# JamesYang007/adelie

Hardware: AMD Instinct MI355X
Metric: lambda-paths/sec (100-lambda grpnet); HBM GB/s vs peak (higher is better)
Workload: dtype f64

## Files before the change

### adelie_amd/csrc/filter_host.hpp

```cpp
#pragma once
#include <algorithm>
#include <cmath>
#include <cstdint>
#include <vector>

namespace ahip {

constexpr int kFilterRuleStrong = 0, kFilterRulePivot = 1;

inline int64_t pivot_need(int64_t old_size, int64_t n_new_active, int64_t G, double subset_ratio, int64_t subset_min,
                          double slack_ratio) {
    const int64_t subset_size =
        std::min<int64_t>(std::max<int64_t>(int64_t(double(old_size) * (1 + subset_ratio)), subset_min), G);
    return subset_size + int64_t(std::ceil(slack_ratio * double(n_new_active))) + old_size + 2;
}

struct FilterRule {
    int screen_rule = kFilterRulePivot;
    double alpha = 1, lm = 0, lm_next = 0;
    bool thr_valid = false;
    double screen_thr = 0;
    int64_t thr_count = 0;
    int64_t G = 0, screen_size = 0, n_new_active = 0;
    double subset_ratio = 0.1, slack_ratio = 1.25;
// ... 8 lines not shown
    } else if (f.screen_rule == kFilterRulePivot) {
        if (!f.thr_valid) return 0;
        if (f.n_new_active > 0) {
            const int64_t need = pivot_need(f.screen_size, f.n_new_active, f.G, f.subset_ratio, f.subset_min, f.slack_ratio);
            if (!(need * 4 < f.G) || double(need) > 0.97 * double(f.thr_count)) return 0;
        }
        tstar = std::min(tstar, f.screen_thr);
    } else {
        return 0;
    }
    return (tstar > 0 && std::isfinite(tstar)) ? tstar : 0;
}

template <class I, class T>
inline std::vector<int32_t> filter_unpenalized_cols(const std::vector<I>& groups, const std::vector<I>& group_sizes,
                                                    const std::vector<T>& penalty) {
    std::vector<int32_t> c;
    for (size_t g = 0; g < groups.size(); ++g)
        if (!(penalty[g] > 0))
            for (I t = 0; t < group_sizes[g]; ++t) c.push_back(int32_t(groups[g] + t));
    return c;
}

constexpr int32_t kFilterOverflow = 1, kFilterStale = 2;
struct FilterFollowUp {
    bool refill;
    bool retire;
};
inline FilterFollowUp filter_follow_up(int32_t flags) {
    return FilterFollowUp{(flags & (kFilterOverflow | kFilterStale)) != 0, (flags & kFilterStale) != 0};
}
inline int64_t filter_list_cap(int64_t p) { return std::max<int64_t>(1024, p / 4); }

}
```

### adelie_amd/csrc/kernels.hpp

```cpp
#pragma once
#include <hip/hip_runtime.h>
#include <cstdint>
#include "gram_shape.hpp"
#include "relu_shape.hpp"
#include "relu_sparse_shape.hpp"
#include "shadow_kind_host.hpp"

namespace ahip {

template <class T>
struct DenseView {
    const T* X;
    int64_t n, p, ld;
};
struct SnpView {
    const uint8_t* bits;
    int64_t n, p, ldb;
};

template <class T>
struct CscView {
    const int64_t* cptr;
    const int32_t* cidx;
    const T* cval;
// ... 28 lines not shown
    const void* X;
    int64_t n, p, ld;
    const double* err;
    const double* nrm;
    int kind = kShadowF32;
    const double* scale = nullptr;
    double fp_term() const { return (4.0 * double(n) + (kind == kShadowQ15 ? 8.0 : 0.0)) * 1.1102230246251565e-16; }
    double elem_bytes() const { return kind == kShadowQ15 ? 2.0 : 4.0; }
};
void launch_shadow_build(const DenseView<double>& X, float* Xs, int64_t lds, double* err, double* nrm, int32_t* bad, hipStream_t s);
int64_t shadow_q15_ld(int64_t n);
void launch_shadow_build_q15(const DenseView<double>& X, int16_t* Xq, int64_t lds, double* scale, double* err, double* nrm,
                             int32_t* bad, hipStream_t s);
int filter_norm_parts(int64_t n);
struct FilteredSweep {
    const double *w, *r;
    double* v;
    double* grad;
    const double *sub_scale, *sub_vec;
    const int32_t* screen_cols;
    int64_t n_screen_cols;
    const int32_t* pen0_cols;
    int64_t n_pen0_cols;
    const int64_t *groups, *group_sizes;
    int64_t G;
    const int32_t* slot;
    const double* penalty;
    double tstar;
    double* sq_part;
    int32_t* list;
    int64_t cap;
    int32_t* meta_i;
    double* meta_d;
    double* work;
};
int64_t filtered_sweep_work_elems(int64_t n, int64_t p, int64_t n_before, int64_t cap);
void enqueue_filtered_sweep(const DenseView<double>& X, const ShadowView& S, const FilteredSweep& a, hipStream_t s);
int64_t sweep_work_elems_csc(int nb, int64_t ncols);
template <class T>
void launch_sweep_csc(const CscView<T>& X, const T* v, T* out, int64_t c0, int64_t ncols, const int32_t* cols,
                      const T* sub_scale, const T* sub_vec, bool square, T* work, hipStream_t s);
constexpr int kVecSumScratch = 8 + 256;
template <class T> void launch_vec_sum(const T* v, int64_t n, T* out, hipStream_t s);
template <class T>
void launch_std_sweep_epilogue(const T* center, const T* inv_scale, const T* raw, const T* raw_plain, const T* vsum, bool square,
                               T* out, int64_t c0, int64_t ncols, const int32_t* cols, const T* sub_scale, const T* sub_vec,
// ... 557 lines not shown
```

### adelie_amd/csrc/kernels_filter.hip

```cpp
#include "sweep_common.hpp"
#include <algorithm>
#include <cfloat>

namespace ahip {

namespace {

__global__ __launch_bounds__(kThreads) void shadow_build_kernel(const double* __restrict__ X, int64_t ld, int64_t n,
                                                                float* __restrict__ Xs, int64_t lds, double* __restrict__ err,
                                                                double* __restrict__ nrm, int32_t* __restrict__ bad) {
    const int64_t j = blockIdx.x;
    const int tid = threadIdx.x;
    const double* col = X + j * ld;
    float* dst = Xs + j * lds;
    double e2 = 0, n2 = 0;
    bool any_bad = false;
    for (int64_t i = tid; i < lds; i += kThreads) {
        float f = 0.f;
        if (i < n) {
            const double x = col[i];
            const bool ok = fabs(x) <= double(FLT_MAX);
            any_bad = any_bad || !ok;
            f = ok ? float(x) : 0.f;
            const double d = x - double(f);
// ... 149 lines not shown

template <int XVEC>
__device__ __forceinline__ void exact_part(const DenseAcc<double>& X, const double* __restrict__ v, int64_t n,
                                           const int32_t* __restrict__ xa, int64_t na, const int32_t* __restrict__ xb,
                                           int64_t nb, int64_t x_rows_per_split, double* __restrict__ stage, double* red) {
    const int64_t ne = na + nb;
    const int64_t c = int64_t(blockIdx.x) % ne;
    const int64_t xsplit = int64_t(blockIdx.x) / ne;
    const int64_t j = c < na ? xa[c] : xb[c - na];
    const int64_t xr0 = xsplit * x_rows_per_split;
    const double s = list_column_sum<XVEC>(X, v, j, xr0, min(n, xr0 + x_rows_per_split), red);
    if (threadIdx.x == 0) stage[xsplit * ne + c] = s;
}

template <class Kind, int XVEC>
__global__ __launch_bounds__(kThreads) void shadow_sweep_kernel(const typename Kind::elem* __restrict__ Xs, int64_t ld,
                                                                const double* __restrict__ scale, const double* __restrict__ v,
                                                                double* __restrict__ out, int64_t n, int64_t ncols,
                                                                int64_t blocks_c, int64_t rows_per_split, int nsplit,
                                                                const double* __restrict__ sub_scale,
                                                                const double* __restrict__ sub_vec, DenseAcc<double> X,
                                                                const int32_t* __restrict__ xa, int64_t na,
                                                                const int32_t* __restrict__ xb, int64_t nb,
                                                                int64_t x_rows_per_split, int x_nsplit, double* __restrict__ stage) {
    constexpr int CB = Kind::CB, VEC = Kind::VEC;
    const int tid = threadIdx.x;
    const int64_t n_exact = (na + nb) * x_nsplit;
    __shared__ double red[kThreads / 64][CB];
    if (int64_t(blockIdx.x) < n_exact) {
        exact_part<XVEC>(X, v, n, xa, na, xb, nb, x_rows_per_split, stage, &red[0][0]);
        return;
    }
    const int64_t b = int64_t(blockIdx.x) - n_exact;
    const int64_t cb = b % blocks_c;
    const int split = int(b / blocks_c);
    const int64_t r0 = int64_t(split) * rows_per_split;
    const int64_t r1 = min(n, r0 + rows_per_split);
    const typename Kind::elem* cp[CB];
#pragma unroll
    for (int k = 0; k < CB; ++k) {
        int64_t c = cb * CB + k;
        if (c >= ncols) c = ncols - 1;
        cp[k] = Xs + c * ld;
    }
    double acc[CB];
#pragma unroll
    for (int k = 0; k < CB; ++k) acc[k] = 0;
    const int64_t body_end = r0 + ((r1 - r0) / VEC) * VEC;
#pragma unroll Kind::kUnroll
    for (int64_t i = r0 + int64_t(tid) * VEC; i < body_end; i += int64_t(kThreads) * VEC) {
        d2_t vv[VEC / 2];
#pragma unroll
        for (int e = 0; e < VEC / 2; ++e) vv[e] = *reinterpret_cast<const d2_t*>(v + i + 2 * e);
        typename Kind::vec xx[CB];
#pragma unroll
        for (int k = 0; k < CB; ++k) xx[k] = __builtin_nontemporal_load(reinterpret_cast<const typename Kind::vec*>(cp[k] + i));
#pragma unroll
        for (int k = 0; k < CB; ++k) {
#pragma unroll
            for (int e = 0; e < VEC; ++e) acc[k] = fma(Kind::row(xx[k], e), vv[e / 2][e % 2], acc[k]);
        }
    }
    for (int64_t i = body_end + tid; i < r1; i += kThreads) {
        const double vi = v[i];
#pragma unroll
        for (int k = 0; k < CB; ++k) acc[k] = fma(double(cp[k][i]), vi, acc[k]);
    }
    panel_epilogue<Kind::kScaled>(acc, red, cb, ncols, 0, nullptr, scale, out, split, nsplit, sub_scale, sub_vec);
}

template <int VEC>
__global__ __launch_bounds__(kThreads) void sweep_list_kernel(DenseAcc<double> X, const double* __restrict__ v,
                                                              double* __restrict__ out, double* __restrict__ part, int64_t n,
                                                              const int32_t* __restrict__ cols, int64_t max_cols,
                                                              const int32_t* __restrict__ count_dev, int64_t rows_per_split,
                                                              int nsplit, const double* __restrict__ sub_scale,
                                                              const double* __restrict__ sub_vec, const double* __restrict__ err,
                                                              const double* __restrict__ nrm, double fp_term,
                                                              const double* __restrict__ vnorm, int32_t* __restrict__ flags) {
    const int64_t c = blockIdx.x;
    const int64_t count = count_dev ? min(int64_t(count_dev[0]), max_cols) : max_cols;
    if (c >= count) return;
    const int split = blockIdx.y;
    const int64_t r0 = int64_t(split) * rows_per_split;
    const int64_t j = cols[c];
    __shared__ double red[kThreads / 64];
    double s = list_column_sum<VEC>(X, v, j, r0, min(n, r0 + rows_per_split), red);
    if (threadIdx.x == 0) {
        if (nsplit == 1) {
            s = centred(s, j, sub_scale, sub_vec);
            if (err) shadow_guard(s, out[j], j, err, nrm, fp_term, vnorm, flags);
// ... 6 lines not shown
__global__ void sweep_list_reduce_kernel(const double* __restrict__ part, double* __restrict__ out,
                                         const int32_t* __restrict__ cols, int64_t max_cols,
                                         const int32_t* __restrict__ count_dev, int nsplit, const double* __restrict__ sub_scale,
                                         const double* __restrict__ sub_vec, const double* __restrict__ err,
                                         const double* __restrict__ nrm, double fp_term, const double* __restrict__ vnorm,
                                         int32_t* __restrict__ flags) {
    const int64_t c = int64_t(blockIdx.x) * blockDim.x + threadIdx.x;
    const int64_t count = count_dev ? min(int64_t(count_dev[0]), max_cols) : max_cols;
    if (c >= count) return;
    const int64_t j = cols[c];
    double s = 0;
    for (int r = 0; r < nsplit; ++r) s += part[int64_t(r) * max_cols + c];
    s = centred(s, j, sub_scale, sub_vec);
    if (err) shadow_guard(s, out[j], j, err, nrm, fp_term, vnorm, flags);
    out[j] = s;
}

constexpr int kClassifyThreads = 1024, kClassifyRun = 6;
__global__ __launch_bounds__(kClassifyThreads) void filter_classify_kernel(
    double* __restrict__ grad, const int64_t* __restrict__ groups, const int64_t* __restrict__ group_sizes, int64_t G,
    const int32_t* __restrict__ slot, const double* __restrict__ penalty, double tstar, const double* __restrict__ err,
    const double* __restrict__ nrm, double fp_term, const double* __restrict__ sq_part, int n_part,
    const double* __restrict__ sub_scale, const double* __restrict__ sub_vec, const double* __restrict__ stage,
    const int32_t* __restrict__ xa, int64_t na, const int32_t* __restrict__ xb, int64_t nb, int x_nsplit,
    int32_t* __restrict__ list, int64_t cap, int32_t* __restrict__ meta_i, double* __restrict__ meta_d) {
    constexpr int NW = kClassifyThreads / 64, R = kClassifyRun;
    __shared__ double sred[NW];
    __shared__ int32_t wtot[NW];
    __shared__ double s_vnorm;
    __shared__ int32_t s_first[kClassifyThreads * R], s_want[kClassifyThreads * R];
    const int tid = threadIdx.x, lane = tid & 63, wv = tid >> 6;
    {
        double a = 0;
        for (int i = tid; i < n_part; i += kClassifyThreads) a += sq_part[i];
        a = wave_sum(a);
        if (lane == 0) sred[wv] = a;
        __syncthreads();
        if (tid == 0) {
            double s = 0;
            for (int w = 0; w < NW; ++w) s += sred[w];
            s_vnorm = sqrt(s) * (1.0 + 1e-6);
            meta_d[0] = s_vnorm;
            meta_d[1] = sub_scale ? sub_scale[0] : 0.0;
            meta_i[1] = 0;
            meta_i[3] = 0;
        }
        __syncthreads();
    }
    const double vnorm = s_vnorm;
    const int64_t ne = na + nb;
    for (int pass = 0; pass < 2; ++pass) {
        const int32_t* xl = pass ? xb : xa;
        const int64_t c0 = pass ? na : 0, cnt = pass ? nb : na;
        for (int64_t c = tid; c < cnt; c += kClassifyThreads) {
            const int64_t j = xl[c];
            double s = 0;
            for (int r = 0; r < x_nsplit; ++r) s += stage[int64_t(r) * ne + c0 + c];
            s = centred(s, j, sub_scale, sub_vec);
            shadow_guard(s, grad[j], j, err, nrm, fp_term, &s_vnorm, meta_i + 1);
            grad[j] = s;
        }
        __syncthreads();
    }
    int64_t run = 0;
    for (int64_t base = 0; base < G; base += int64_t(kClassifyThreads) * R) {
        int32_t k[R], sz[R];
        double thr[R], a2[R], b2[R];
        {
            int32_t sl[R];
            double pn[R];
            int64_t kk[R], ss[R];
#pragma unroll
            for (int u = 0; u < R; ++u) {
                const int64_t gu = base + int64_t(u) * kClassifyThreads + tid;
                const int64_t g = gu < G ? gu : G - 1;
                sl[u] = slot[g];
                pn[u] = penalty[g];
                kk[u] = groups[g];
                ss[u] = group_sizes[g];
            }
#pragma unroll
            for (int u = 0; u < R; ++u) {
// ... 110 lines not shown
    if (L.ns > 1)
        hipLaunchKernelGGL(sweep_list_reduce_kernel, dim3((unsigned)((max_cols + 255) / 256)), dim3(256), 0, s, work, out, cols,
                           max_cols, count_dev, L.ns, sub_scale, sub_vec, guard.err, guard.nrm, guard.fp_term(), vnorm, flags);
}
int64_t shadow_work_elems(int64_t n, int64_t p) {
    int64_t blocks_c, rps;
    int ns, ns16;
    sweep_shape(n, p, kShadowVec, blocks_c, ns, rps, kShadowCB);
    sweep_shape(n, p, kShadowVec16, blocks_c, ns16, rps, kShadowCB16);
    return int64_t(std::max(ns, ns16)) * p + 16;
}
int64_t list_work_elems(int64_t n, int64_t p, int64_t max_cols) {
    int64_t blocks_c, rps;
    int ns;
    sweep_shape(n, p, 1, blocks_c, ns, rps);
    return int64_t(ns) * max_cols + 16;
}
template <class Kind, int XVEC>
void launch_shadow_sweep(const DenseView<double>& X, const ShadowView& S, const FilteredSweep& a, int64_t na, int64_t nb,
                         const ListShape& L, double* stage, hipStream_t s) {
    int64_t blocks_c, rps;
    int ns;
    sweep_shape(S.n, S.p, Kind::VEC, blocks_c, ns, rps, Kind::CB);
    hipLaunchKernelGGL((shadow_sweep_kernel<Kind, XVEC>), dim3((unsigned)((na + nb) * L.ns + blocks_c * ns)), dim3(kThreads), 0, s,
                       static_cast<const typename Kind::elem*>(S.X), S.ld, S.scale, a.v, ns == 1 ? a.grad : a.work, S.n, S.p,
                       blocks_c, rps, ns, a.sub_scale, a.sub_vec, DenseAcc<double>{X.X, X.ld}, a.screen_cols, na, a.pen0_cols, nb,
                       L.rps, L.ns, stage);
    if (ns > 1) launch_sweep_reduce<double>(a.work, a.grad, S.p, ns, 0, nullptr, a.sub_scale, a.sub_vec, s);
}
}

int64_t filtered_sweep_work_elems(int64_t n, int64_t p, int64_t n_before, int64_t cap) {
    return shadow_work_elems(n, p) + list_work_elems(n, p, std::max(n_before, cap));
}
void enqueue_filtered_sweep(const DenseView<double>& X, const ShadowView& S, const FilteredSweep& a, hipStream_t s) {
    if (S.p <= 0) return;
    const int64_t na = a.screen_cols ? a.n_screen_cols : 0, nb = a.pen0_cols ? a.n_pen0_cols : 0;
    double* stage = a.work + shadow_work_elems(S.n, S.p);
    hipLaunchKernelGGL(vmul_sq_kernel, dim3(grid1d(S.n, kThreads, 1024)), dim3(kThreads), 0, s, a.w, a.r, a.v, S.n, a.sq_part);
    const ListShape L = list_shape(X, a.v);
    constexpr int V = VecOf<double>::N;
    if (S.kind == kShadowQ15) {
        if (L.vec) launch_shadow_sweep<ShadowQ15, V>(X, S, a, na, nb, L, stage, s);
        else launch_shadow_sweep<ShadowQ15, 1>(X, S, a, na, nb, L, stage, s);
    } else {
        if (L.vec) launch_shadow_sweep<ShadowF32, V>(X, S, a, na, nb, L, stage, s);
        else launch_shadow_sweep<ShadowF32, 1>(X, S, a, na, nb, L, stage, s);
    }
    hipLaunchKernelGGL(filter_classify_kernel, dim3(1), dim3(kClassifyThreads), 0, s, a.grad, a.groups, a.group_sizes, a.G, a.slot,
                       a.penalty, a.tstar, S.err, S.nrm, S.fp_term(), a.sq_part, filter_norm_parts(S.n), a.sub_scale, a.sub_vec,
                       stage, a.screen_cols, na, a.pen0_cols, nb, L.ns, a.list, a.cap, a.meta_i, a.meta_d);
    launch_sweep_list(X, a.v, a.grad, a.list, a.cap, a.meta_i, a.sub_scale, a.sub_vec, S, a.meta_d, a.meta_i + 1, stage, s);
}

}
```

### adelie_amd/csrc/screen_reads_host.hpp

```cpp
#pragma once
#include "filter_host.hpp"
#include <limits>
#include <utility>

namespace ahip {

template <class T>
inline int search_pivot(const std::vector<T>& x, const std::vector<T>& y, std::vector<T>& mses) {
    const int64_t m = int64_t(x.size());
    if (m <= 0) return -1;
    mses[0] = std::numeric_limits<T>::infinity();
    if (m == 1) return 0;
    T y_mean = 0;
    for (int64_t i = 0; i < m; ++i) y_mean += y[i];
    y_mean /= T(m);
    T x_sum = x[0], xsq_sum = x[0] * x[0], y_sum = y[0], yx_sum = y[0] * x[0], min_mse = mses[0];
    int argmin = 0;
    for (int64_t i = 1; i < m; ++i) {
        x_sum += x[i];
        xsq_sum += x[i] * x[i];
        y_sum += y[i];
        yx_sum += y[i] * x[i];
        const T t_bar = ((i + 1) * x[i] - x_sum) / m;
        const T var_t = ((i + 1) * x[i] * x[i] - 2 * x[i] * x_sum + xsq_sum - m * t_bar * t_bar);
// ... 51 lines not shown
        ++count;
    }
    return r;
}


constexpr double kDepthMargin = 0.25;
constexpr int64_t kDepthExtra = 16;
inline int64_t pivot_subset_size(int64_t screen_size, int64_t G, double subset_ratio, int64_t subset_min) {
    return std::min<int64_t>(std::max<int64_t>(int64_t(double(screen_size) * (1 + subset_ratio)), subset_min), G);
}
inline int64_t predict_reads(int64_t subset_next, int64_t last_reads, int64_t last_subset, int64_t n_new_active,
                             double slack_ratio) {
    const int64_t walk = last_reads > 0 ? std::max<int64_t>(last_reads - last_subset, 0)
                                        : 2 * int64_t(std::ceil(slack_ratio * double(std::max<int64_t>(n_new_active, 1))));
    return subset_next + walk;
}
inline int64_t filter_depth(int64_t G, int64_t reads_pred, double m) {
    if (G <= 0) return 0;
    const double d = std::ceil((1 + std::max(m, 0.0)) * double(std::max<int64_t>(reads_pred, 0)));
    const int64_t D = (d < double(G) ? int64_t(d) : G) + (m > 0 ? kDepthExtra : 0);
    return std::max<int64_t>(1, std::min<int64_t>(G, D));
}
template <class T>
inline T depth_score(std::vector<T>& scores, int64_t D) {
    const int64_t G = int64_t(scores.size());
    if (G == 0) return std::numeric_limits<T>::infinity();
    D = std::max<int64_t>(1, std::min<int64_t>(D, G));
    std::nth_element(scores.begin(), scores.begin() + (D - 1), scores.end(), std::greater<T>());
    return scores[size_t(D - 1)];
}

template <class T>
inline T depth_score_hinted(const std::vector<T>& scores, int64_t D, T lo_hint, std::vector<T>& scratch) {
    const int64_t G = int64_t(scores.size());
    D = std::max<int64_t>(1, std::min<int64_t>(D, G));
    scratch.clear();
    if (lo_hint > 0)
        for (const T s : scores)
            if (s >= lo_hint) scratch.push_back(s);
    if (int64_t(scratch.size()) < D) scratch = scores;
    return depth_score(scratch, D);
}

#ifndef AHIP_FILTER_BYTES_RHO
#define AHIP_FILTER_BYTES_RHO 0.6
#endif
constexpr double kFilterBytesRho = AHIP_FILTER_BYTES_RHO;
constexpr double kFilterBytesRuleMin = double(int64_t(1) << 28);
inline bool filter_bytes_eligible(int64_t exact_cols, int64_t n, int64_t p, int64_t skip_cols, double shadow_elem_bytes,
                                  double rho = kFilterBytesRho) {
    if (p <= 0 || n <= 0) return false;
    const double full = 8.0 * double(n) * double(p);
    if (full < kFilterBytesRuleMin) return true;
    const double bytes = double(n) * (8.0 * double(std::max<int64_t>(exact_cols, 0)) +
                                      shadow_elem_bytes * double(std::max<int64_t>(p - std::max<int64_t>(skip_cols, 0), 0)));
    return bytes < rho * full;
}
inline int64_t filter_depth_list_cap(int64_t p) { return std::max<int64_t>(1024, p / 2); }

}
```

### adelie_amd/csrc/solver.hip

```cpp
#include "common.hpp"
#include "design_ops.hpp"
#include "filter_host.hpp"
#include "screen_reads_host.hpp"
#include "cox.hpp"

#include <algorithm>
#include <cstring>
#include <exception>
#include <type_traits>
#include <chrono>
#include <condition_variable>
#include <mutex>
#include <thread>
#include <cmath>
#include <cstdio>
#include <cstdlib>
#include <limits>
#include <numeric>
#include <unordered_set>

namespace ahip {
void set_last_error(const std::string& s);
double g_hessian_min = 1e-24;
double g_dbeta_tol = 1e-12;
// ... 771 lines not shown
    try {
        if (!d || !w || !r || !groups || !group_sizes || !penalty || !grad || !exact || !info || G < 1 || n_screen < 0)
            throw make_core_error("bad arguments.");
        if (!d->is_dense() || d->dtype != ADELIE_HIP_F64 || d->cov || d->constraint || d->std_center) throw make_core_error("a dense f64 design is required.");
        AHIP_CHECK(hipSetDevice(d->device));
        hipStream_t s = d->stream;
        const int64_t n = d->n, p = d->p;
        if (groups[G - 1] + group_sizes[G - 1] != p) throw make_core_error("groups do not cover the columns.");
        std::vector<int32_t> slot(size_t(G), -1), scols, pen0;
        for (int64_t k = 0; k < n_screen; ++k) {
            const int64_t g = screen_groups[k];
            if (g < 0 || g >= G) throw make_core_error("screen group out of range.");
            slot[size_t(g)] = int32_t(scols.size());
            for (int64_t t = 0; t < group_sizes[g]; ++t) scols.push_back(int32_t(groups[g] + t));
        }
        for (int64_t g = 0; g < G; ++g)
            if (!(penalty[g] > 0))
                for (int64_t t = 0; t < group_sizes[g]; ++t) pen0.push_back(int32_t(groups[g] + t));
        ShadowView sh{};
        const bool route = filter_sweep_on(Hooks::filter_sweep_env()) && adelie_hip_internal_shadow_acquire(d, &sh);
        const int64_t cap = filter_list_cap(p);
        DevBuf<double> dw, dr, dv, dgrad, dxm, dsc, dpen, dpart, dmetad, work;
        DevBuf<int64_t> dgroups, dgs;
        DevBuf<int32_t> dslot, dscols, dpen0, dlist, dmeta;
        dw.reserve(n); dr.reserve(n); dv.reserve(n); dgrad.reserve(p); dsc.reserve(1); dpen.reserve(G); dgroups.reserve(G);
        dgs.reserve(G); dslot.reserve(G); dlist.reserve(cap); dmeta.reserve(4); dmetad.reserve(2);
        const int n_part = filter_norm_parts(n);
        dpart.reserve(n_part);
        work.reserve(size_t(std::max(filtered_sweep_work_elems(n, p, int64_t(scols.size() + pen0.size()), cap), sweep_work_elems(n, p))));
        dw.upload(w, n, s); dr.upload(r, n, s); dsc.upload(&sub_scale, 1, s); dpen.upload(penalty, G, s);
        dgroups.upload(groups, G, s); dgs.upload(group_sizes, G, s); dslot.upload(slot.data(), G, s);
        if (sub_vec) { dxm.reserve(p); dxm.upload(sub_vec, p, s); }
        if (!scols.empty()) { dscols.reserve(scols.size()); dscols.upload(scols.data(), scols.size(), s); }
        if (!pen0.empty()) { dpen0.reserve(pen0.size()); dpen0.upload(pen0.data(), pen0.size(), s); }
        const double* xm = sub_vec ? dxm.p : nullptr;
        const DenseView<double> X = d->dense<double>();
        int32_t meta[4] = {0, 0, 0, 0};
        std::vector<int32_t> list;
        if (!route) {
            launch_vmul<double>(dw.p, dr.p, dv.p, n, s);
            launch_sweep<double>(X, dv.p, dgrad.p, 0, p, nullptr, dsc.p, xm, false, work.p, s);
            std::fill(exact, exact + p, uint8_t(1));
        } else {
            FilteredSweep a{};
            a.w = dw.p; a.r = dr.p; a.v = dv.p; a.grad = dgrad.p; a.sub_scale = dsc.p; a.sub_vec = xm;
            a.screen_cols = scols.empty() ? nullptr : dscols.p; a.n_screen_cols = int64_t(scols.size());
            a.pen0_cols = pen0.empty() ? nullptr : dpen0.p; a.n_pen0_cols = int64_t(pen0.size());
            a.groups = dgroups.p; a.group_sizes = dgs.p; a.G = G; a.slot = dslot.p; a.penalty = dpen.p; a.tstar = tstar;
            a.sq_part = dpart.p; a.list = dlist.p; a.cap = cap; a.meta_i = dmeta.p; a.meta_d = dmetad.p; a.work = work.p;
            enqueue_filtered_sweep(X, sh, a, s);
            AHIP_CHECK(hipMemcpyAsync(meta, dmeta.p, sizeof(meta), hipMemcpyDeviceToHost, s));
            AHIP_CHECK(hipStreamSynchronize(s));
            list.resize(size_t(meta[0]));
            if (meta[0] > 0) AHIP_CHECK(hipMemcpyAsync(list.data(), dlist.p, size_t(meta[0]) * sizeof(int32_t), hipMemcpyDeviceToHost, s));
            std::fill(exact, exact + p, uint8_t(0));
        }
        AHIP_CHECK(hipMemcpyAsync(grad, dgrad.p, size_t(p) * sizeof(double), hipMemcpyDeviceToHost, s));
        AHIP_CHECK(hipStreamSynchronize(s));
        if (route) {
            for (int32_t c : scols) exact[c] = 1;
            for (int32_t c : pen0) exact[c] = 1;
            for (int32_t c : list) exact[c] = 1;
            if (meta[1] & 2) adelie_hip_internal_shadow_mark_stale(d);
        }
        info[0] = meta[0]; info[1] = meta[1]; info[2] = route ? 1 : 0; info[3] = meta[2];
    } catch (const std::exception& e) {
        set_last_error(e.what());
        return 1;
    }
    return 0;
// ... 369 lines not shown
```

### adelie_amd/csrc/solver_screen.hpp

```cpp
    void sweep(const T* v, T* out, const int32_t* cols, idx ncols, const T* sub_scale, const T* sub_vec,
               bool square = false) {
        if (multi()) {
            if (cols || ncols != p || sub_vec || square) throw make_core_error("unsupported sweep on a multi-response view.");
            const MultiView<T> mv = D->multi<T>();
            launch_multi_sweep<T>(mv, v, out, d_work_sweep.reserve(size_t(multi_sweep_work_elems<T>(mv))), st);
            return;
        }
        if (std_generic()) {
            const T* ce = static_cast<const T*>(D->std_center);
            const T* is = static_cast<const T*>(D->std_iscale);
            T* tmp = d_std_tmp.reserve(size_t(2 * ncols + kVecSumScratch));
            T *raw = tmp, *raw_plain = tmp + ncols, *vsum = tmp + 2 * ncols;
            T* work = d_work_sweep.reserve(size_t(raw_sweep_work_elems(*D, ncols, false)));
            raw_sweep<T>(*D, v, raw, 0, ncols, cols, nullptr, nullptr, square, false, work, st);
            if (square) raw_sweep<T>(*D, v, raw_plain, 0, ncols, cols, nullptr, nullptr, false, false, work, st);
            launch_vec_sum<T>(v, n, vsum, st);
            launch_std_sweep_epilogue<T>(ce, is, raw, raw_plain, vsum, square, out, 0, ncols, cols, sub_scale, sub_vec, st);
            return;
        }
        if (batcher && dense() && !cols && ncols == p && !square &&
            batcher->template sweep<T>(D->dense<T>(), v, out, sub_scale, sub_vec, st)) {
            ++cnt.n_sweeps_shared;
            return;
        }
// ... 249 lines not shown
                                        d_grad.p, d_beta.p, d_penalty.p, (1 - alpha) * lm, d_cons_va.p, d_cons_vb.p, d_cons_mu.p, d_absgrad.p, st);
        } else {
            launch_abs_grad<T>(d_grad.p, d_groups.p, d_gsizes.p, G, d_slot.p, d_beta.p, has_pen2 ? d_penalty2.p : d_penalty.p,
                               (1 - alpha) * lm, d_absgrad.p, st);
        }
        d_absgrad.download(abs_grad.data(), size_t(G), st);
    }

    int fs_state = 0;
    ShadowView fs_shadow{};
    bool grad_filtered = false;
    T inv_next_lm = 0;
    int solve_active_size = 0;
    int64_t screen_thr_count = 0;
    T fs_lm = 0;
    DevBuf<int32_t> d_fs_list, d_fs_meta, d_fs_pen0;
    DevBuf<T> d_fs_part, d_fs_metad, d_fs_work, d_fs_v, d_fs_abs;
    int64_t fs_pen0_cols = -1;
    int32_t fs_meta[4] = {0, 0, 0, 0};
    std::vector<T> fs_abs_host;
    KTimer t_fsweep;
    double fsweep_bytes = 0;
    int64_t n_sweeps_filtered = 0, n_sweeps_refilled = 0, n_filter_exact_cols = 0, n_filter_shadow_cols = 0;
    int64_t fs_pending_screen_cols = 0;
    int64_t fs_cap() const { return depth_rule() ? filter_depth_list_cap(int64_t(p)) : filter_list_cap(int64_t(p)); }

    bool filter_eligible() const {
        if constexpr (!std::is_same<T, double>::value) return false;
        if (!filter_sweep_on(hooks.filter_sweep)) return false;
        if (!dense() || is_glm() || cov_mode || cons_on || multi() || std_generic() || batcher || D->factor() || has_pen2) return false;
        if (D->relu() && relu_sweep_on(hooks.relu_sweep)) return false;
        return true;
    }

    bool depth_rule() const {
        return fs_state >= 0 && filter_depth_on(hooks.filter_depth) && screen_rule == ADELIE_HIP_SCREEN_PIVOT && filter_eligible();
    }
    bool depth_thr_valid = false;
    int64_t depth_pen0_cols = -1;
    int64_t depth_open_cols = 0;
    int64_t depth_last_reads = 0, depth_last_subset = 0;
    int64_t n_screen_reads = 0, n_screen_short = 0, n_filter_open_cols = 0;
    std::vector<T> depth_scores, depth_scratch;
    bool depth_scores_fresh = false;
    std::vector<idx> screen_append;

    void set_depth_threshold(int n_new_active) {
        if (!depth_rule()) return;
        const int64_t Gi = int64_t(G);
        if (fs_state == 1 && !filter_bytes_eligible(int64_t(screen_beta.size()) + std::max<int64_t>(depth_pen0_cols, 0), int64_t(n),
                                                    int64_t(p), 0, double(fs_shadow.elem_bytes()))) {
            depth_thr_valid = false;
            depth_scores_fresh = false;
            return;
        }
        const int64_t subset_next =
            pivot_subset_size(int64_t(screen_set.size()), Gi, double(pivot_subset_ratio), int64_t(pivot_subset_min));
        const int64_t reads_pred =
            predict_reads(subset_next, depth_last_reads, depth_last_subset, int64_t(n_new_active), double(pivot_slack_ratio));
        const double m = hooks.filter_depth_margin >= 0 ? hooks.filter_depth_margin : kDepthMargin;
        const int64_t Dp = filter_depth(Gi, reads_pred, m);
        if (!depth_scores_fresh) {
            depth_scores.resize(size_t(Gi));
            for (idx i = 0; i < G; ++i) depth_scores[size_t(i)] = pivot_score(i);
        }
        depth_scores_fresh = false;
        screen_thr = depth_score_hinted(depth_scores, Dp, depth_thr_valid ? T(0.9) * screen_thr : T(0), depth_scratch);
        depth_thr_valid = Gi > 0;
        depth_open_cols = 0;
        for (idx i = 0; i < G; ++i)
            if (depth_scores[size_t(i)] >= screen_thr && !is_screen(i) && penalty[i] > 0) depth_open_cols += group_sizes[i];
        if (hooks.trace)
            std::fprintf(stderr, "[depth] lmda %.6g |S| %lld subset_next %lld reads_pred %lld D %lld thr %.9g open_cols %lld\n",
                         double(lmda), (long long)screen_set.size(), (long long)subset_next, (long long)reads_pred, (long long)Dp,
                         double(screen_thr), (long long)depth_open_cols);
    }

    T filter_threshold(T lm, int active_now) {
        if (fs_state < 0 || !filter_eligible()) return T(0);
        if (depth_rule()) {
            if (!depth_thr_valid || !(inv_next_lm > 0) || !(lm > 0) || !(alpha > 0)) return T(0);
            const T tstar = std::min(std::min(alpha * lm, alpha * inv_next_lm), screen_thr);
            if (!(tstar > 0) || !std::isfinite(tstar)) return T(0);
            if (depth_pen0_cols < 0) depth_pen0_cols = int64_t(filter_unpenalized_cols(groups, group_sizes, penalty).size());
            if (depth_open_cols + depth_open_cols / 8 > fs_cap()) return T(0);
            if (fs_state == 0) fs_state = adelie_hip_internal_shadow_acquire(D, &fs_shadow) ? 1 : -1;
            if (fs_state != 1) return T(0);
            const int64_t exact = int64_t(nv) + depth_pen0_cols + depth_open_cols;
            return filter_bytes_eligible(exact, int64_t(n), int64_t(p), 0, double(fs_shadow.elem_bytes())) ? tstar : T(0);
        }
        FilterRule f;
        f.screen_rule = screen_rule == ADELIE_HIP_SCREEN_STRONG ? kFilterRuleStrong
                        : screen_rule == ADELIE_HIP_SCREEN_PIVOT ? kFilterRulePivot : -1;
        f.alpha = double(alpha); f.lm = double(lm); f.lm_next = double(inv_next_lm);
        f.thr_valid = screen_thr_valid; f.screen_thr = double(screen_thr); f.thr_count = screen_thr_count;
        f.G = int64_t(G); f.screen_size = int64_t(screen_set.size());
        f.n_new_active = std::max(0, active_now - solve_active_size);
        f.subset_ratio = double(pivot_subset_ratio); f.subset_min = int64_t(pivot_subset_min); f.slack_ratio = double(pivot_slack_ratio);
        const T tstar = T(filter_tstar(f));
        if (!(tstar > 0)) return T(0);
        if (fs_state == 0) fs_state = adelie_hip_internal_shadow_acquire(D, &fs_shadow) ? 1 : -1;
        return fs_state == 1 ? tstar : T(0);
    }

    void invariance_sweep(T lm, int active_now, const T* rsum_dev) {
        const T tstar = filter_threshold(lm, active_now);
        if (!(tstar > 0)) {
            launch_vmul<T>(d_w.p, d_r.p, d_v.p, n, st);
            t_sweep.begin(st);
            sweep(d_v.p, d_grad.p, nullptr, p, rsum_dev, intercept ? d_xm.p : nullptr);
            t_sweep.end(st);
            grad_filtered = false;
            return;
        }
        if constexpr (std::is_same<T, double>::value) {
            const T* xm = intercept ? d_xm.p : nullptr;
            const int64_t cap = fs_cap();
            if (fs_pen0_cols < 0) {
                const std::vector<int32_t> c0 = filter_unpenalized_cols(groups, group_sizes, penalty);
                fs_pen0_cols = int64_t(c0.size());
                if (!c0.empty()) {
                    d_fs_pen0.reserve(c0.size());
                    d_fs_pen0.upload(c0.data(), c0.size(), st);
                }
            }
            d_fs_part.reserve(size_t(filter_norm_parts(n)));
            d_fs_meta.reserve(4);
            d_fs_metad.reserve(2);
            d_fs_list.reserve(size_t(cap));
            d_fs_work.reserve(size_t(filtered_sweep_work_elems(n, p, int64_t(nv) + fs_pen0_cols, cap)));
            FilteredSweep a{};
            a.w = d_w.p; a.r = d_r.p; a.v = d_v.p; a.grad = d_grad.p; a.sub_scale = rsum_dev; a.sub_vec = xm;
            a.screen_cols = nv > 0 ? d_vcol.p : nullptr; a.n_screen_cols = nv;
            a.pen0_cols = fs_pen0_cols > 0 ? d_fs_pen0.p : nullptr; a.n_pen0_cols = fs_pen0_cols;
            a.groups = d_groups.p; a.group_sizes = d_gsizes.p; a.G = G; a.slot = d_slot.p; a.penalty = d_penalty.p; a.tstar = tstar;
            a.sq_part = d_fs_part.p; a.list = d_fs_list.p; a.cap = cap; a.meta_i = d_fs_meta.p; a.meta_d = d_fs_metad.p;
            a.work = d_fs_work.p;
            t_fsweep.begin(st);
            enqueue_filtered_sweep(D->dense<T>(), fs_shadow, a, st);
            t_fsweep.end(st);
            d_fs_meta.download(fs_meta, 4, st);
            grad_filtered = true;
            fs_lm = lm;
            fs_pending_screen_cols = int64_t(nv) + std::max<int64_t>(fs_pen0_cols, 0);
            ++n_sweeps_filtered;
        }
    }

    void filtered_sweep_arrived() {
        if (!grad_filtered) return;
        const int64_t exact = fs_pending_screen_cols + fs_meta[0];
        n_filter_exact_cols += exact;
        n_filter_open_cols += fs_meta[0];
        if (hooks.trace)
            std::fprintf(stderr, "[fsweep] lmda %.6g screen+pen0 cols %lld open %d wanted %d flags %d predicted open %lld\n",
                         double(fs_lm), (long long)fs_pending_screen_cols, int(fs_meta[0]), int(fs_meta[2]), int(fs_meta[1]),
                         (long long)depth_open_cols);
        n_filter_shadow_cols += int64_t(p);
        fsweep_bytes += double(n) * (double(exact) * 8.0 + double(p) * fs_shadow.elem_bytes());
        const FilterFollowUp fu = filter_follow_up(fs_meta[1]);
        if (fu.retire) {
            adelie_hip_internal_shadow_mark_stale(D);
            fs_state = -1;
        }
        if (fu.refill) ensure_exact_grad();
    }

    void ensure_exact_grad() {
        if (!grad_filtered) return;
        grad_filtered = false;
        ++n_sweeps_refilled;
        const T* rsrc = spec_active ? d_r_snap.p : d_r.p;
        d_fs_v.reserve(size_t(n));
        d_fs_abs.reserve(size_t(G));
        launch_vmul<T>(d_w.p, rsrc, d_fs_v.p, n, st);
        t_sweep.begin(st);
        sweep(d_fs_v.p, d_grad.p, nullptr, p, d_fs_metad.p + 1, intercept ? d_xm.p : nullptr);
        t_sweep.end(st);
        launch_abs_grad<T>(d_grad.p, d_groups.p, d_gsizes.p, G, d_slot.p, d_beta.p, d_penalty.p, (1 - alpha) * fs_lm, d_fs_abs.p, st);
        fs_abs_host.resize(size_t(G));
        d_fs_abs.download(fs_abs_host.data(), size_t(G), st);
        sync();
// ... 570 lines not shown
```

### adelie_amd/csrc/sweep_common.hpp

```cpp
#pragma once
#include "kernels.hpp"
#include "accessors.hpp"
#include "sweep_shape.hpp"

namespace ahip {

template <class T>
void launch_sweep_reduce(const T* part, T* out, int64_t ncols, int nsplit, int64_t c0, const int32_t* cols, const T* sub_scale,
                         const T* sub_vec, hipStream_t s);

namespace {

constexpr int kThreads = 256;
static_assert(kThreads == kSweepThreads, "sweep_shape.hpp counts rows per iteration of a kThreads workgroup");

template <class T>
__device__ __forceinline__ T wave_sum(T x) {
#pragma unroll
    for (int off = 32; off > 0; off >>= 1) x += __shfl_down(x, off, 64);
    return x;
}

template <class T, int VEC>
__device__ __forceinline__ Pack<T, VEC> load_vec(const T* p) {
// ... 14 lines not shown
    return (X.ld % V == 0) && ((reinterpret_cast<uintptr_t>(X.X) % 16) == 0);
}

inline unsigned grid1d(int64_t n, int bt, int64_t cap = 4096) {
    int64_t g = (n + bt - 1) / bt;
    if (g > cap) g = cap;
    if (g < 1) g = 1;
    return unsigned(g);
}

template <class T>
__device__ __forceinline__ T centred(T s, int64_t j, const T* sub_scale, const T* sub_vec) {
    if (sub_vec) s -= sub_scale[0] * sub_vec[j];
    return s;
}

template <class T>
__device__ __forceinline__ void store_sum(T s, T* out, int64_t c, int64_t j, int split, int nsplit, int64_t stride,
                                          const T* sub_scale, const T* sub_vec) {
    if (nsplit == 1) out[c] = centred(s, j, sub_scale, sub_vec);
    else out[int64_t(split) * stride + c] = s;
}

template <bool SCALED, class T, int CB>
__device__ __forceinline__ void panel_epilogue(const T (&acc)[CB], T (&red)[kThreads / 64][CB], int64_t cb, int64_t ncols,
                                               int64_t c0, const int32_t* cols, const double* scale, T* out, int split,
                                               int nsplit, const T* sub_scale, const T* sub_vec) {
    const int tid = threadIdx.x, lane = tid & 63, wv = tid >> 6;
#pragma unroll
    for (int k = 0; k < CB; ++k) {
        const T s = wave_sum(acc[k]);
        if (lane == 0) red[wv][k] = s;
    }
    __syncthreads();
    if (tid < CB) {
        const int64_t c = cb * CB + tid;
        if (c < ncols) {
            T s = T(0);
#pragma unroll
            for (int w = 0; w < kThreads / 64; ++w) s += red[w][tid];
            if constexpr (SCALED) s = __dmul_rn(s, scale[c]);
            store_sum(s, out, c, cols ? int64_t(cols[c]) : c0 + c, split, nsplit, ncols, sub_scale, sub_vec);
        }
    }
}

}
}
```

Before: 4.952.

## Skip shadow sweep over screened and unpenalized columns already computed exactly

The filtered sweep now builds a host-side list of columns that excludes screen and unpenalized columns, keeping a small guard sample of screen columns. The low-precision shadow sweep runs only over that list, with a scatter epilogue and a list-based reduce. The change avoids reading those columns twice, once in shadow precision and once exactly. It also relaxes the byte-eligibility threshold and depth rule so filtering is chosen more often. The cost is a host rebuild and upload of the column list whenever the screen set changes, and the shadow guard now checks only the sampled columns.

Result: faster. 5.044, median of 6 (+1.9%).

```diff
diff --git a/adelie_amd/csrc/filter_host.hpp b/adelie_amd/csrc/filter_host.hpp
--- a/adelie_amd/csrc/filter_host.hpp
+++ b/adelie_amd/csrc/filter_host.hpp
@@ -54,6 +54,29 @@
     return c;
 }
 
+constexpr int64_t kFilterGuardSample = 64;
+inline void filter_shadow_cols(int64_t p, const int32_t* screen_cols, int64_t n_screen, const int32_t* pen0_cols, int64_t n_pen0,
+                               std::vector<uint8_t>& mark, std::vector<int32_t>& out) {
+    mark.assign(size_t(std::max<int64_t>(p, 0)), 0);
+    out.clear();
+    auto set = [&](int32_t c, uint8_t to) { if (c >= 0 && int64_t(c) < p) mark[size_t(c)] = to; };
+    for (int64_t i = 0; i < n_pen0; ++i) set(pen0_cols[i], 1);
+    for (int64_t i = 0; i < n_screen; ++i) set(screen_cols[i], 1);
+    for (int64_t i = 0; i < std::min(n_screen, kFilterGuardSample); ++i) set(screen_cols[i], 0);
+    out.resize(mark.size());
+    size_t k = 0;
+    for (int64_t c = 0; c < p; ++c) {
+        out[k] = int32_t(c);
+        k += size_t(mark[size_t(c)] == 0);
+    }
+    out.resize(k);
+}
+constexpr int64_t kFilterListStale = 256;
+inline int64_t filter_shadow_skip(int64_t n_screen, int64_t n_pen0) {
+    return std::max<int64_t>(n_screen, 0) + std::max<int64_t>(n_pen0, 0) -
+           std::min<int64_t>(std::max<int64_t>(n_screen, 0), kFilterGuardSample);
+}
+
 constexpr int32_t kFilterOverflow = 1, kFilterStale = 2;
 struct FilterFollowUp {
     bool refill;
diff --git a/adelie_amd/csrc/kernels.hpp b/adelie_amd/csrc/kernels.hpp
--- a/adelie_amd/csrc/kernels.hpp
+++ b/adelie_amd/csrc/kernels.hpp
@@ -74,6 +74,8 @@
     int64_t n_screen_cols;
     const int32_t* pen0_cols;
     int64_t n_pen0_cols;
+    const int32_t* shadow_cols;
+    int64_t n_shadow_cols;
     const int64_t *groups, *group_sizes;
     int64_t G;
     const int32_t* slot;
diff --git a/adelie_amd/csrc/kernels_filter.hip b/adelie_amd/csrc/kernels_filter.hip
--- a/adelie_amd/csrc/kernels_filter.hip
+++ b/adelie_amd/csrc/kernels_filter.hip
@@ -1,4 +1,5 @@
 #include "sweep_common.hpp"
+#include "filter_host.hpp"
 #include <algorithm>
 #include <cfloat>
 
@@ -195,7 +196,8 @@
                                                                 const double* __restrict__ sub_vec, DenseAcc<double> X,
                                                                 const int32_t* __restrict__ xa, int64_t na,
                                                                 const int32_t* __restrict__ xb, int64_t nb,
-                                                                int64_t x_rows_per_split, int x_nsplit, double* __restrict__ stage) {
+                                                                int64_t x_rows_per_split, int x_nsplit, double* __restrict__ stage,
+                                                                const int32_t* __restrict__ scols) {
     constexpr int CB = Kind::CB, VEC = Kind::VEC;
     const int tid = threadIdx.x;
     const int64_t n_exact = (na + nb) * x_nsplit;
@@ -214,7 +216,7 @@
     for (int k = 0; k < CB; ++k) {
         int64_t c = cb * CB + k;
         if (c >= ncols) c = ncols - 1;
-        cp[k] = Xs + c * ld;
+        cp[k] = Xs + (scols ? int64_t(scols[c]) : c) * ld;
     }
     double acc[CB];
 #pragma unroll
@@ -239,7 +241,8 @@
 #pragma unroll
         for (int k = 0; k < CB; ++k) acc[k] = fma(double(cp[k][i]), vi, acc[k]);
     }
-    panel_epilogue<Kind::kScaled>(acc, red, cb, ncols, 0, nullptr, scale, out, split, nsplit, sub_scale, sub_vec);
+    if (!scols) panel_epilogue<Kind::kScaled>(acc, red, cb, ncols, 0, nullptr, scale, out, split, nsplit, sub_scale, sub_vec);
+    else panel_epilogue<Kind::kScaled, true>(acc, red, cb, ncols, 0, scols, scale, out, split, nsplit, sub_scale, sub_vec);
 }
 
 template <int VEC>
@@ -292,8 +295,8 @@
     const int32_t* __restrict__ slot, const double* __restrict__ penalty, double tstar, const double* __restrict__ err,
     const double* __restrict__ nrm, double fp_term, const double* __restrict__ sq_part, int n_part,
     const double* __restrict__ sub_scale, const double* __restrict__ sub_vec, const double* __restrict__ stage,
-    const int32_t* __restrict__ xa, int64_t na, const int32_t* __restrict__ xb, int64_t nb, int x_nsplit,
-    int32_t* __restrict__ list, int64_t cap, int32_t* __restrict__ meta_i, double* __restrict__ meta_d) {
+    const int32_t* __restrict__ xa, int64_t na, const int32_t* __restrict__ xb, int64_t nb, int x_nsplit, int64_t na_guard,
+    int64_t nb_guard, int32_t* __restrict__ list, int64_t cap, int32_t* __restrict__ meta_i, double* __restrict__ meta_d) {
     constexpr int NW = kClassifyThreads / 64, R = kClassifyRun;
     __shared__ double sred[NW];
     __shared__ int32_t wtot[NW];
@@ -321,13 +324,13 @@
     const int64_t ne = na + nb;
     for (int pass = 0; pass < 2; ++pass) {
         const int32_t* xl = pass ? xb : xa;
-        const int64_t c0 = pass ? na : 0, cnt = pass ? nb : na;
+        const int64_t c0 = pass ? na : 0, cnt = pass ? nb : na, guarded = pass ? nb_guard : na_guard;
         for (int64_t c = tid; c < cnt; c += kClassifyThreads) {
             const int64_t j = xl[c];
             double s = 0;
             for (int r = 0; r < x_nsplit; ++r) s += stage[int64_t(r) * ne + c0 + c];
             s = centred(s, j, sub_scale, sub_vec);
-            shadow_guard(s, grad[j], j, err, nrm, fp_term, &s_vnorm, meta_i + 1);
+            if (c < guarded) shadow_guard(s, grad[j], j, err, nrm, fp_term, &s_vnorm, meta_i + 1);
             grad[j] = s;
         }
         __syncthreads();
@@ -484,11 +487,20 @@
     int64_t blocks_c, rps;
     int ns;
     sweep_shape(S.n, S.p, Kind::VEC, blocks_c, ns, rps, Kind::CB);
-    hipLaunchKernelGGL((shadow_sweep_kernel<Kind, XVEC>), dim3((unsigned)((na + nb) * L.ns + blocks_c * ns)), dim3(kThreads), 0, s,
-                       static_cast<const typename Kind::elem*>(S.X), S.ld, S.scale, a.v, ns == 1 ? a.grad : a.work, S.n, S.p,
+    const int64_t ncols = a.shadow_cols ? a.n_shadow_cols : S.p;
+    blocks_c = (ncols + Kind::CB - 1) / Kind::CB;
+    const int64_t grid = (na + nb) * L.ns + blocks_c * ns;
+    if (grid <= 0) return;
+    hipLaunchKernelGGL((shadow_sweep_kernel<Kind, XVEC>), dim3((unsigned)grid), dim3(kThreads), 0, s,
+                       static_cast<const typename Kind::elem*>(S.X), S.ld, S.scale, a.v, ns == 1 ? a.grad : a.work, S.n, ncols,
                        blocks_c, rps, ns, a.sub_scale, a.sub_vec, DenseAcc<double>{X.X, X.ld}, a.screen_cols, na, a.pen0_cols, nb,
-                       L.rps, L.ns, stage);
-    if (ns > 1) launch_sweep_reduce<double>(a.work, a.grad, S.p, ns, 0, nullptr, a.sub_scale, a.sub_vec, s);
+                       L.rps, L.ns, stage, a.shadow_cols);
+    if (ns > 1 && ncols > 0) {
+        if (!a.shadow_cols) launch_sweep_reduce<double>(a.work, a.grad, S.p, ns, 0, nullptr, a.sub_scale, a.sub_vec, s);
+        else
+            hipLaunchKernelGGL(sweep_list_reduce_kernel, dim3((unsigned)((ncols + 255) / 256)), dim3(256), 0, s, a.work, a.grad,
+                               a.shadow_cols, ncols, nullptr, ns, a.sub_scale, a.sub_vec, nullptr, nullptr, 0.0, nullptr, nullptr);
+    }
 }
 }
 
@@ -497,6 +509,12 @@
 }
 void enqueue_filtered_sweep(const DenseView<double>& X, const ShadowView& S, const FilteredSweep& a, hipStream_t s) {
     if (S.p <= 0) return;
+    if (a.shadow_cols && a.n_shadow_cols >= S.p) {
+        FilteredSweep all = a;
+        all.shadow_cols = nullptr;
+        enqueue_filtered_sweep(X, S, all, s);
+        return;
+    }
     const int64_t na = a.screen_cols ? a.n_screen_cols : 0, nb = a.pen0_cols ? a.n_pen0_cols : 0;
     double* stage = a.work + shadow_work_elems(S.n, S.p);
     hipLaunchKernelGGL(vmul_sq_kernel, dim3(grid1d(S.n, kThreads, 1024)), dim3(kThreads), 0, s, a.w, a.r, a.v, S.n, a.sq_part);
@@ -511,7 +529,9 @@
     }
     hipLaunchKernelGGL(filter_classify_kernel, dim3(1), dim3(kClassifyThreads), 0, s, a.grad, a.groups, a.group_sizes, a.G, a.slot,
                        a.penalty, a.tstar, S.err, S.nrm, S.fp_term(), a.sq_part, filter_norm_parts(S.n), a.sub_scale, a.sub_vec,
-                       stage, a.screen_cols, na, a.pen0_cols, nb, L.ns, a.list, a.cap, a.meta_i, a.meta_d);
+                       stage, a.screen_cols, na, a.pen0_cols, nb, L.ns,
+                       a.shadow_cols ? std::min<int64_t>(na, kFilterGuardSample) : na, a.shadow_cols ? int64_t(0) : nb, a.list, a.cap,
+                       a.meta_i, a.meta_d);
     launch_sweep_list(X, a.v, a.grad, a.list, a.cap, a.meta_i, a.sub_scale, a.sub_vec, S, a.meta_d, a.meta_i + 1, stage, s);
 }
 
diff --git a/adelie_amd/csrc/screen_reads_host.hpp b/adelie_amd/csrc/screen_reads_host.hpp
--- a/adelie_amd/csrc/screen_reads_host.hpp
+++ b/adelie_amd/csrc/screen_reads_host.hpp
@@ -97,6 +97,19 @@
     const int64_t D = (d < double(G) ? int64_t(d) : G) + (m > 0 ? kDepthExtra : 0);
     return std::max<int64_t>(1, std::min<int64_t>(G, D));
 }
+constexpr double kDepthOutsideMargin = 0.5;
+constexpr int64_t kDepthOutsideFloor = 32;
+inline int64_t filter_depth_outside(int64_t G, int64_t reads_pred, int64_t screen_size, double m) {
+    if (G <= 0) return 0;
+    const int64_t r = std::min<int64_t>(std::max<int64_t>(reads_pred, 0), G);
+    int64_t D = r;
+    if (m > 0) {
+        const double extra = std::ceil(m * double(std::max<int64_t>(r - std::max<int64_t>(screen_size, 0), 0)));
+        const int64_t add = std::max<int64_t>(extra < double(G) ? int64_t(extra) : G, kDepthOutsideFloor);
+        D = add >= G - r ? G : r + add;
+    }
+    return std::max<int64_t>(1, D);
+}
 template <class T>
 inline T depth_score(std::vector<T>& scores, int64_t D) {
     const int64_t G = int64_t(scores.size());
@@ -132,6 +145,10 @@
                                       shadow_elem_bytes * double(std::max<int64_t>(p - std::max<int64_t>(skip_cols, 0), 0)));
     return bytes < rho * full;
 }
+#ifndef AHIP_FILTER_BYTES_RHO_READ
+#define AHIP_FILTER_BYTES_RHO_READ 0.7
+#endif
+constexpr double kFilterBytesRhoRead = AHIP_FILTER_BYTES_RHO_READ;
 inline int64_t filter_depth_list_cap(int64_t p) { return std::max<int64_t>(1024, p / 2); }
 
 }
diff --git a/adelie_amd/csrc/solver.hip b/adelie_amd/csrc/solver.hip
--- a/adelie_amd/csrc/solver.hip
+++ b/adelie_amd/csrc/solver.hip
@@ -817,7 +817,10 @@
         const int64_t cap = filter_list_cap(p);
         DevBuf<double> dw, dr, dv, dgrad, dxm, dsc, dpen, dpart, dmetad, work;
         DevBuf<int64_t> dgroups, dgs;
-        DevBuf<int32_t> dslot, dscols, dpen0, dlist, dmeta;
+        DevBuf<int32_t> dslot, dscols, dpen0, dlist, dmeta, dshadow;
+        std::vector<uint8_t> mark;
+        std::vector<int32_t> shadow_cols;
+        filter_shadow_cols(p, scols.data(), int64_t(scols.size()), pen0.data(), int64_t(pen0.size()), mark, shadow_cols);
         dw.reserve(n); dr.reserve(n); dv.reserve(n); dgrad.reserve(p); dsc.reserve(1); dpen.reserve(G); dgroups.reserve(G);
         dgs.reserve(G); dslot.reserve(G); dlist.reserve(cap); dmeta.reserve(4); dmetad.reserve(2);
         const int n_part = filter_norm_parts(n);
@@ -828,6 +831,8 @@
         if (sub_vec) { dxm.reserve(p); dxm.upload(sub_vec, p, s); }
         if (!scols.empty()) { dscols.reserve(scols.size()); dscols.upload(scols.data(), scols.size(), s); }
         if (!pen0.empty()) { dpen0.reserve(pen0.size()); dpen0.upload(pen0.data(), pen0.size(), s); }
+        dshadow.reserve(std::max<size_t>(shadow_cols.size(), 1));
+        dshadow.upload(shadow_cols.data(), shadow_cols.size(), s);
         const double* xm = sub_vec ? dxm.p : nullptr;
         const DenseView<double> X = d->dense<double>();
         int32_t meta[4] = {0, 0, 0, 0};
@@ -841,6 +846,7 @@
             a.w = dw.p; a.r = dr.p; a.v = dv.p; a.grad = dgrad.p; a.sub_scale = dsc.p; a.sub_vec = xm;
             a.screen_cols = scols.empty() ? nullptr : dscols.p; a.n_screen_cols = int64_t(scols.size());
             a.pen0_cols = pen0.empty() ? nullptr : dpen0.p; a.n_pen0_cols = int64_t(pen0.size());
+            a.shadow_cols = dshadow.p; a.n_shadow_cols = int64_t(shadow_cols.size());
             a.groups = dgroups.p; a.group_sizes = dgs.p; a.G = G; a.slot = dslot.p; a.penalty = dpen.p; a.tstar = tstar;
             a.sq_part = dpart.p; a.list = dlist.p; a.cap = cap; a.meta_i = dmeta.p; a.meta_d = dmetad.p; a.work = work.p;
             enqueue_filtered_sweep(X, sh, a, s);
diff --git a/adelie_amd/csrc/solver_screen.hpp b/adelie_amd/csrc/solver_screen.hpp
--- a/adelie_amd/csrc/solver_screen.hpp
+++ b/adelie_amd/csrc/solver_screen.hpp
@@ -295,7 +295,11 @@
     KTimer t_fsweep;
     double fsweep_bytes = 0;
     int64_t n_sweeps_filtered = 0, n_sweeps_refilled = 0, n_filter_exact_cols = 0, n_filter_shadow_cols = 0;
-    int64_t fs_pending_screen_cols = 0;
+    int64_t fs_pending_screen_cols = 0, fs_pending_shadow_cols = 0;
+    DevBuf<int32_t> d_fs_shadow;
+    std::vector<int32_t> fs_shadow_host, fs_shadow_from, fs_pen0_host;
+    std::vector<uint8_t> fs_shadow_mark;
+    bool fs_shadow_valid = false;
     int64_t fs_cap() const { return depth_rule() ? filter_depth_list_cap(int64_t(p)) : filter_list_cap(int64_t(p)); }
 
     bool filter_eligible() const {
@@ -321,8 +325,10 @@
     void set_depth_threshold(int n_new_active) {
         if (!depth_rule()) return;
         const int64_t Gi = int64_t(G);
-        if (fs_state == 1 && !filter_bytes_eligible(int64_t(screen_beta.size()) + std::max<int64_t>(depth_pen0_cols, 0), int64_t(n),
-                                                    int64_t(p), 0, double(fs_shadow.elem_bytes()))) {
+        const int64_t pen0 = std::max<int64_t>(depth_pen0_cols, 0);
+        if (fs_state == 1 && !filter_bytes_eligible(int64_t(screen_beta.size()) + pen0, int64_t(n), int64_t(p),
+                                                    filter_shadow_skip(int64_t(screen_beta.size()), pen0),
+                                                    double(fs_shadow.elem_bytes()), kFilterBytesRhoRead)) {
             depth_thr_valid = false;
             depth_scores_fresh = false;
             return;
@@ -331,8 +337,8 @@
             pivot_subset_size(int64_t(screen_set.size()), Gi, double(pivot_subset_ratio), int64_t(pivot_subset_min));
         const int64_t reads_pred =
             predict_reads(subset_next, depth_last_reads, depth_last_subset, int64_t(n_new_active), double(pivot_slack_ratio));
-        const double m = hooks.filter_depth_margin >= 0 ? hooks.filter_depth_margin : kDepthMargin;
-        const int64_t Dp = filter_depth(Gi, reads_pred, m);
+        const double m = hooks.filter_depth_margin >= 0 ? hooks.filter_depth_margin : kDepthOutsideMargin;
+        const int64_t Dp = filter_depth_outside(Gi, reads_pred, int64_t(screen_set.size()), m);
         if (!depth_scores_fresh) {
             depth_scores.resize(size_t(Gi));
             for (idx i = 0; i < G; ++i) depth_scores[size_t(i)] = pivot_score(i);
@@ -360,7 +366,9 @@
             if (fs_state == 0) fs_state = adelie_hip_internal_shadow_acquire(D, &fs_shadow) ? 1 : -1;
             if (fs_state != 1) return T(0);
             const int64_t exact = int64_t(nv) + depth_pen0_cols + depth_open_cols;
-            return filter_bytes_eligible(exact, int64_t(n), int64_t(p), 0, double(fs_shadow.elem_bytes())) ? tstar : T(0);
+            return filter_bytes_eligible(exact, int64_t(n), int64_t(p), filter_shadow_skip(int64_t(nv), depth_pen0_cols),
+                                         double(fs_shadow.elem_bytes()), kFilterBytesRhoRead)
+                       ? tstar : T(0);
         }
         FilterRule f;
         f.screen_rule = screen_rule == ADELIE_HIP_SCREEN_STRONG ? kFilterRuleStrong
@@ -390,12 +398,25 @@
             const T* xm = intercept ? d_xm.p : nullptr;
             const int64_t cap = fs_cap();
             if (fs_pen0_cols < 0) {
-                const std::vector<int32_t> c0 = filter_unpenalized_cols(groups, group_sizes, penalty);
+                fs_pen0_host = filter_unpenalized_cols(groups, group_sizes, penalty);
+                const std::vector<int32_t>& c0 = fs_pen0_host;
                 fs_pen0_cols = int64_t(c0.size());
                 if (!c0.empty()) {
                     d_fs_pen0.reserve(c0.size());
                     d_fs_pen0.upload(c0.data(), c0.size(), st);
                 }
+                fs_shadow_valid = false;
+            }
+            if (h_vcol.size() < size_t(nv)) throw make_core_error("filtered sweep: the host mirror of the screen columns is short.");
+            if (!fs_shadow_valid || fs_shadow_from.size() > size_t(nv) ||
+                int64_t(nv) - int64_t(fs_shadow_from.size()) >= kFilterListStale ||
+                !std::equal(fs_shadow_from.begin(), fs_shadow_from.end(), h_vcol.begin())) {
+                fs_shadow_from.assign(h_vcol.begin(), h_vcol.begin() + nv);
+                filter_shadow_cols(int64_t(p), fs_shadow_from.data(), int64_t(nv), fs_pen0_host.data(), fs_pen0_cols, fs_shadow_mark,
+                                   fs_shadow_host);
+                d_fs_shadow.reserve(size_t(std::max<idx>(p, 1)));
+                d_fs_shadow.upload(fs_shadow_host.data(), fs_shadow_host.size(), st);
+                fs_shadow_valid = true;
             }
             d_fs_part.reserve(size_t(filter_norm_parts(n)));
             d_fs_meta.reserve(4);
@@ -406,6 +427,7 @@
             a.w = d_w.p; a.r = d_r.p; a.v = d_v.p; a.grad = d_grad.p; a.sub_scale = rsum_dev; a.sub_vec = xm;
             a.screen_cols = nv > 0 ? d_vcol.p : nullptr; a.n_screen_cols = nv;
             a.pen0_cols = fs_pen0_cols > 0 ? d_fs_pen0.p : nullptr; a.n_pen0_cols = fs_pen0_cols;
+            a.shadow_cols = d_fs_shadow.p; a.n_shadow_cols = int64_t(fs_shadow_host.size());
             a.groups = d_groups.p; a.group_sizes = d_gsizes.p; a.G = G; a.slot = d_slot.p; a.penalty = d_penalty.p; a.tstar = tstar;
             a.sq_part = d_fs_part.p; a.list = d_fs_list.p; a.cap = cap; a.meta_i = d_fs_meta.p; a.meta_d = d_fs_metad.p;
             a.work = d_fs_work.p;
@@ -416,6 +438,7 @@
             grad_filtered = true;
             fs_lm = lm;
             fs_pending_screen_cols = int64_t(nv) + std::max<int64_t>(fs_pen0_cols, 0);
+            fs_pending_shadow_cols = int64_t(fs_shadow_host.size());
             ++n_sweeps_filtered;
         }
     }
@@ -429,8 +452,8 @@
             std::fprintf(stderr, "[fsweep] lmda %.6g screen+pen0 cols %lld open %d wanted %d flags %d predicted open %lld\n",
                          double(fs_lm), (long long)fs_pending_screen_cols, int(fs_meta[0]), int(fs_meta[2]), int(fs_meta[1]),
                          (long long)depth_open_cols);
-        n_filter_shadow_cols += int64_t(p);
-        fsweep_bytes += double(n) * (double(exact) * 8.0 + double(p) * fs_shadow.elem_bytes());
+        n_filter_shadow_cols += fs_pending_shadow_cols;
+        fsweep_bytes += double(n) * (double(exact) * 8.0 + double(fs_pending_shadow_cols) * fs_shadow.elem_bytes());
         const FilterFollowUp fu = filter_follow_up(fs_meta[1]);
         if (fu.retire) {
             adelie_hip_internal_shadow_mark_stale(D);
diff --git a/adelie_amd/csrc/sweep_common.hpp b/adelie_amd/csrc/sweep_common.hpp
--- a/adelie_amd/csrc/sweep_common.hpp
+++ b/adelie_amd/csrc/sweep_common.hpp
@@ -60,7 +60,7 @@
     else out[int64_t(split) * stride + c] = s;
 }
 
-template <bool SCALED, class T, int CB>
+template <bool SCALED, bool SCATTER = false, class T, int CB>
 __device__ __forceinline__ void panel_epilogue(const T (&acc)[CB], T (&red)[kThreads / 64][CB], int64_t cb, int64_t ncols,
                                                int64_t c0, const int32_t* cols, const double* scale, T* out, int split,
                                                int nsplit, const T* sub_scale, const T* sub_vec) {
@@ -77,8 +77,10 @@
             T s = T(0);
 #pragma unroll
             for (int w = 0; w < kThreads / 64; ++w) s += red[w][tid];
-            if constexpr (SCALED) s = __dmul_rn(s, scale[c]);
-            store_sum(s, out, c, cols ? int64_t(cols[c]) : c0 + c, split, nsplit, ncols, sub_scale, sub_vec);
+            const int64_t j = cols ? int64_t(cols[c]) : c0 + c;
+            if constexpr (SCALED) s = __dmul_rn(s, scale[SCATTER ? j : c]);
+            if (SCATTER && nsplit == 1) out[j] = centred(s, j, sub_scale, sub_vec);
+            else store_sum(s, out, c, j, split, nsplit, ncols, sub_scale, sub_vec);
         }
     }
 }
```
